# retab-dev/k-LLMs

Hardware: AMD Instinct MI355X
Metric: end_to_end_consensus_requests_per_s (higher is better)
Workload: dtype bf16; 1 GPU; model=llama-3-8b, n=5, mode=create, global_batch=24, seq_len=512, parallelism=dp1 tp1

## Files before the change

### kllms_amd/ops/hip/attn_decode.hip

```cpp

#include "common.h"

#define TKV ATTN_DECODE_TKV
#define NTHREADS 256
#define KLANES 4

#define PART_STRIDE 130

template <int GQA, bool FP8>
__global__ __launch_bounds__(NTHREADS) void attn_decode_partial_t(
    float* __restrict__ partials,
    const bf16_t* __restrict__ q,
    const char* __restrict__ k_cache,
    const char* __restrict__ v_cache,
    const float* __restrict__ k_scale,
    const float* __restrict__ v_scale,
    const int* __restrict__ block_tables,
    const int* __restrict__ context_lens,
    const int* __restrict__ skip_chunks,
    float scale, int num_kv_heads,
    int block_size, int max_blocks, int max_chunks, int q_tstride, int chunk_keys) {
  const int b = blockIdx.x;
  const int g_kv = blockIdx.y;
  const int chunk = blockIdx.z;
  if (skip_chunks != nullptr && chunk < skip_chunks[b]) return;
  const int L = context_lens[b];
  const int c0 = chunk * chunk_keys;
  if (c0 >= L && chunk > 0) return;
  const int c1 = min(L, c0 + chunk_keys);
  const int tid = threadIdx.x;

  extern __shared__ __attribute__((aligned(16))) char smem[];
  float* q_lds = reinterpret_cast<float*>(smem);
  float* s_lds = q_lds + GQA * 128;
  float* mstate = s_lds + GQA * TKV;
  float* lstate = mstate + 8;
  float* alpha_lds = lstate + 8;
  float* o_scratch = alpha_lds + 8;
  int64_t* rowoff = reinterpret_cast<int64_t*>(o_scratch + 4 * GQA * 128);
  float* ks_lds = reinterpret_cast<float*>(rowoff + TKV);
  float* vs_lds = ks_lds + TKV;

  for (int i = tid; i < GQA * 128; i += NTHREADS) {
    const int g = i >> 7, d = i & 127;
    const bf16_t* qp = q + (int64_t)b * q_tstride + (g_kv * GQA + g) * 128;
    q_lds[i] = bf16_to_f32(((const short*)qp)[d]) * scale;
  }
  if (tid < 8) { mstate[tid] = -INFINITY; lstate[tid] = 0.0f; }
  __syncthreads();

  float o_part[GQA][2];
#pragma unroll
  for (int g = 0; g < GQA; ++g) { o_part[g][0] = 0.f; o_part[g][1] = 0.f; }

  const int* bt = block_tables + (int64_t)b * max_blocks;

  for (int tile = c0; tile < c1; tile += TKV) {
    const int nkeys = min(TKV, c1 - tile);
    for (int i = tid; i < nkeys; i += NTHREADS) {
      const int gk = tile + i;
      const int64_t off = (((int64_t)bt[gk / block_size] * num_kv_heads + g_kv) * block_size +
                           (gk % block_size)) * 128;
      rowoff[i] = off;
      if constexpr (FP8) {
        ks_lds[i] = k_scale[off >> 7];
        vs_lds[i] = v_scale[off >> 7];
      }
    }
    __syncthreads();

    {
      constexpr int ELEMS = 128 / KLANES;
      constexpr int VECS = ELEMS / 8;
      const int kg = tid / KLANES;
      const int kl = tid % KLANES;
      for (int key0 = 0; key0 < nkeys; key0 += NTHREADS / KLANES) {
        const int key = key0 + kg;
        if (key < nkeys) {
          float af[ELEMS];
          if constexpr (FP8) {
            const u8x8_vec* kv8 = reinterpret_cast<const u8x8_vec*>(k_cache + rowoff[key]) + kl * VECS;
#pragma unroll
            for (int c = 0; c < VECS; ++c) {
              u8x8_vec kv = kv8[c];
#pragma unroll
              for (int j = 0; j < 8; ++j) af[c * 8 + j] = fp8_to_f32(kv[j]);
            }
          } else {
            const bf16x8_vec* kv8 =
                reinterpret_cast<const bf16x8_vec*>(k_cache + 2 * rowoff[key]) + kl * VECS;
#pragma unroll
            for (int c = 0; c < VECS; ++c) {
              bf16x8_vec kv = kv8[c];
#pragma unroll
              for (int j = 0; j < 8; ++j) af[c * 8 + j] = bf16_to_f32(kv[j]);
            }
          }
#pragma unroll
          for (int g = 0; g < GQA; ++g) {
            const float* qg = q_lds + g * 128 + kl * ELEMS;
            float acc = 0.f;
#pragma unroll
            for (int j = 0; j < ELEMS; ++j) acc += af[j] * qg[j];
#pragma unroll
            for (int off = KLANES / 2; off > 0; off >>= 1) acc += __shfl_xor(acc, off);
            if (kl == 0) s_lds[g * TKV + key] = FP8 ? acc * ks_lds[key] : acc;
          }
        }
      }
    }
    __syncthreads();

    {
      const int wave = tid >> 6;
      const int wlane = tid & 63;
      for (int g = wave; g < GQA; g += NTHREADS / 64) {
        float lm = -INFINITY;
        for (int i = wlane; i < nkeys; i += 64) lm = fmaxf(lm, s_lds[g * TKV + i]);
        const float tile_max = wave_reduce_max(lm);
        const float m_old = mstate[g];
        const float m_new = fmaxf(m_old, tile_max);
        const float alpha = (m_old == -INFINITY) ? 0.0f : __expf(m_old - m_new);
        float ls = 0.f;
        for (int i = wlane; i < nkeys; i += 64) {
          const float p = __expf(s_lds[g * TKV + i] - m_new);
          s_lds[g * TKV + i] = p;
          ls += p;
        }
        const float tile_sum = wave_reduce_sum(ls);
        if (wlane == 0) {
          alpha_lds[g] = alpha;
          mstate[g] = m_new;
          lstate[g] = lstate[g] * alpha + tile_sum;
        }
      }
    }
    __syncthreads();

    {
      const int kpart = tid >> 6;
      const int d0 = (tid & 63) * 2;
#pragma unroll
      for (int g = 0; g < GQA; ++g) {
        const float alpha = alpha_lds[g];
        o_part[g][0] *= alpha;
        o_part[g][1] *= alpha;
      }
      const int nk4 = (nkeys + 3) >> 2;
      const int kbeg = kpart * nk4;
      const int kend = min(nkeys, kbeg + nk4);
      int key = kbeg;
      for (; key + 4 <= kend; key += 4) {
        uint32_t pairs[4];
#pragma unroll
        for (int u = 0; u < 4; ++u) {
          if constexpr (FP8)
            pairs[u] = *reinterpret_cast<const unsigned short*>(v_cache + rowoff[key + u] + d0);
          else
            pairs[u] = *reinterpret_cast<const uint32_t*>(v_cache + 2 * (rowoff[key + u] + d0));
        }
#pragma unroll
        for (int u = 0; u < 4; ++u) {
          const float vs = FP8 ? vs_lds[key + u] : 1.0f;
          const float v0 = vs * (FP8 ? fp8_to_f32((unsigned char)(pairs[u] & 0xff))
                                     : bf16_to_f32((short)(pairs[u] & 0xffff)));
          const float v1 = vs * (FP8 ? fp8_to_f32((unsigned char)((pairs[u] >> 8) & 0xff))
                                     : bf16_to_f32((short)(pairs[u] >> 16)));
#pragma unroll
          for (int g = 0; g < GQA; ++g) {
            const float p = s_lds[g * TKV + key + u];
            o_part[g][0] += p * v0;
            o_part[g][1] += p * v1;
          }
        }
      }
      for (; key < kend; ++key) {
        uint32_t pair;
        if constexpr (FP8)
          pair = *reinterpret_cast<const unsigned short*>(v_cache + rowoff[key] + d0);
        else
          pair = *reinterpret_cast<const uint32_t*>(v_cache + 2 * (rowoff[key] + d0));
        const float vs = FP8 ? vs_lds[key] : 1.0f;
        const float v0 = vs * (FP8 ? fp8_to_f32((unsigned char)(pair & 0xff))
                                   : bf16_to_f32((short)(pair & 0xffff)));
        const float v1 = vs * (FP8 ? fp8_to_f32((unsigned char)((pair >> 8) & 0xff))
                                   : bf16_to_f32((short)(pair >> 16)));
#pragma unroll
        for (int g = 0; g < GQA; ++g) {
          const float p = s_lds[g * TKV + key];
          o_part[g][0] += p * v0;
          o_part[g][1] += p * v1;
        }
      }
    }
    __syncthreads();
  }

  {
    const int kpart = tid >> 6;
    const int d0 = (tid & 63) * 2;
#pragma unroll
    for (int g = 0; g < GQA; ++g) {
      o_scratch[((kpart * GQA + g) * 128) + d0] = o_part[g][0];
      o_scratch[((kpart * GQA + g) * 128) + d0 + 1] = o_part[g][1];
    }
  }
  __syncthreads();
  float* base = partials +
      ((((int64_t)b * num_kv_heads + g_kv) * max_chunks + chunk) * GQA) * PART_STRIDE;
  for (int i = tid; i < GQA * 128; i += NTHREADS) {
    const int g = i >> 7, d = i & 127;
    float acc = 0.f;
#pragma unroll
    for (int kp = 0; kp < 4; ++kp) acc += o_scratch[((kp * GQA + g) * 128) + d];
    base[g * PART_STRIDE + d] = acc;
  }
  if (tid < 8 && tid < GQA) {
    float* pg = base + tid * PART_STRIDE;
    pg[128] = mstate[tid];
    pg[129] = lstate[tid];
  }
}

extern "C" void launch_attn_decode_partial(
    float* partials, const bf16_t* q, const void* k_cache, const void* v_cache,
    const float* k_scale, const float* v_scale,
    const int* block_tables, const int* context_lens, const int* skip_chunks, float scale,
    int num_q_heads, int num_kv_heads, int block_size, int max_blocks,
    int max_chunks, int q_tstride, int chunk_keys, int B, int cache_fp8,
    hipStream_t stream) {
  const int gqa = num_q_heads / num_kv_heads;
  const dim3 grid(B, num_kv_heads, max_chunks);
  const size_t lds = (gqa * 128 + gqa * TKV + 24 + 4 * gqa * 128) * sizeof(float) +
                     TKV * sizeof(int64_t) + 2 * TKV * sizeof(float);
#define LAUNCH(G, F)                                                                  \
  hipLaunchKernelGGL((attn_decode_partial_t<G, F>), grid, dim3(NTHREADS), lds, stream, \
                     partials, q, (const char*)k_cache, (const char*)v_cache,          \
                     k_scale, v_scale,                                                 \
                     block_tables, context_lens, skip_chunks, scale, num_kv_heads,     \
                     block_size,                                                       \
                     max_blocks, max_chunks, q_tstride, chunk_keys)
#define DISPATCH(G) do { if (cache_fp8) LAUNCH(G, true); else LAUNCH(G, false); } while (0)
  switch (gqa) {
    case 1: DISPATCH(1); break;
    case 2: DISPATCH(2); break;
    case 4: DISPATCH(4); break;
    case 8: DISPATCH(8); break;
    default: DISPATCH(8); break;
  }
#undef DISPATCH
#undef LAUNCH
}

extern "C" __global__ void __launch_bounds__(64) attn_decode_reduce_kernel(
    bf16_t* __restrict__ out,
    const float* __restrict__ partials,
    const int* __restrict__ context_lens,
    int num_q_heads, int num_kv_heads, int max_chunks, int chunk_keys) {
  const int b = blockIdx.x;
  const int h = blockIdx.y;
  const int gqa = num_q_heads / num_kv_heads;
  const int g_kv = h / gqa;
  const int g = h % gqa;
  const int lane = threadIdx.x;
  const int nchunks = min(max_chunks, (context_lens[b] + chunk_keys - 1) / chunk_keys);

  const float* base = partials +
      ((((int64_t)b * num_kv_heads + g_kv) * max_chunks) * gqa + g) * PART_STRIDE;

  float m = -INFINITY;
  for (int c = 0; c < nchunks; ++c) m = fmaxf(m, base[(int64_t)c * gqa * PART_STRIDE + 128]);
  float l_tot = 0.0f;
  float acc0 = 0.0f, acc1 = 0.0f;
  for (int c = 0; c < nchunks; ++c) {
    const float* pc = base + (int64_t)c * gqa * PART_STRIDE;
    const float w = __expf(pc[128] - m);
    l_tot += pc[129] * w;
    acc0 += pc[lane * 2] * w;
    acc1 += pc[lane * 2 + 1] * w;
  }
  const float inv_l = (l_tot > 0.f) ? 1.0f / l_tot : 0.0f;
  bf16_t* op = out + (((int64_t)b * num_q_heads) + h) * 128;
  const uint32_t pair = ((uint32_t)(uint16_t)f32_to_bf16(acc1 * inv_l) << 16) |
                        (uint16_t)f32_to_bf16(acc0 * inv_l);
  *reinterpret_cast<uint32_t*>((short*)op + lane * 2) = pair;
}
```

Baseline: 31.08 req/s.

## Prefetch V rows in groups, swizzle block order, and use DPP quad reductions in decode attention

The P·V loop now loads V in groups of 16 keys and double-buffers them, so the next group's global loads are in flight while the current group's FMAs run. The blocks are also changed: the launch grid is linearised and batches are swizzled across groups of 8, the q load is vectorised and overlapped with first-tile rowoff staging (dropping one barrier), the key-lane reduction uses DPP instead of shuffles, and launch bounds request 4 blocks per SM. The extra registers for two 16-entry buffers may hurt occupancy or spill. Selective non-contracted multiply-add keeps rounding behaviour matched for the last GQA group.

```diff
diff --git a/kllms_amd/ops/hip/attn_decode.hip b/kllms_amd/ops/hip/attn_decode.hip
--- a/kllms_amd/ops/hip/attn_decode.hip
+++ b/kllms_amd/ops/hip/attn_decode.hip
@@ -1,14 +1,33 @@
 
 #include "common.h"
+
+#include <type_traits>
 
 #define TKV ATTN_DECODE_TKV
 #define NTHREADS 256
 #define KLANES 4
 
 #define PART_STRIDE 130
+#define V_GROUP 16
+
+static_assert(TKV == NTHREADS, "one rowoff slot per thread");
+
+__device__ __forceinline__ float quad_sum(float acc) {
+  acc += __int_as_float(__builtin_amdgcn_update_dpp(
+      0, __float_as_int(acc), 0x4E , 0xF, 0xF, false));
+  acc += __int_as_float(__builtin_amdgcn_update_dpp(
+      0, __float_as_int(acc), 0xB1 , 0xF, 0xF, false));
+  return acc;
+}
+
+__device__ __forceinline__ float mul_then_add(float p, float v, float o) {
+#pragma clang fp contract(off)
+  const float pv = p * v;
+  return o + pv;
+}
 
 template <int GQA, bool FP8>
-__global__ __launch_bounds__(NTHREADS) void attn_decode_partial_t(
+__global__ __launch_bounds__(NTHREADS, 4) void attn_decode_partial_t(
     float* __restrict__ partials,
     const bf16_t* __restrict__ q,
     const char* __restrict__ k_cache,
@@ -20,9 +39,25 @@
     const int* __restrict__ skip_chunks,
     float scale, int num_kv_heads,
     int block_size, int max_blocks, int max_chunks, int q_tstride, int chunk_keys) {
-  const int b = blockIdx.x;
-  const int g_kv = blockIdx.y;
-  const int chunk = blockIdx.z;
+  int b, g_kv, chunk;
+  {
+    const int nb = gridDim.x, ny = gridDim.y;
+    const int nb8 = nb / 8;
+    const int swizzled = nb8 * 8 * ny * (int)gridDim.z;
+    const int lin = blockIdx.x + nb * (blockIdx.y + ny * blockIdx.z);
+    int rest;
+    if (lin < swizzled) {
+      const int idx = lin / 8;
+      b = (lin % 8) * nb8 + idx % nb8;
+      rest = idx / nb8;
+    } else {
+      const int r = lin - swizzled, tail = nb - 8 * nb8;
+      b = 8 * nb8 + r % tail;
+      rest = r / tail;
+    }
+    g_kv = rest % ny;
+    chunk = rest / ny;
+  }
   if (skip_chunks != nullptr && chunk < skip_chunks[b]) return;
   const int L = context_lens[b];
   const int c0 = chunk * chunk_keys;
@@ -41,32 +76,45 @@
   float* ks_lds = reinterpret_cast<float*>(rowoff + TKV);
   float* vs_lds = ks_lds + TKV;
 
-  for (int i = tid; i < GQA * 128; i += NTHREADS) {
-    const int g = i >> 7, d = i & 127;
-    const bf16_t* qp = q + (int64_t)b * q_tstride + (g_kv * GQA + g) * 128;
-    q_lds[i] = bf16_to_f32(((const short*)qp)[d]) * scale;
+  const int* bt = block_tables + (int64_t)b * max_blocks;
+  auto stage_rowoff = [&](int tile, int nkeys) {
+    if (tid < nkeys) {
+      const int gk = tile + tid;
+      const int64_t off = (((int64_t)bt[gk / block_size] * num_kv_heads + g_kv) * block_size +
+                           (gk % block_size)) * 128;
+      rowoff[tid] = off;
+      if constexpr (FP8) {
+        ks_lds[tid] = k_scale[off >> 7];
+        vs_lds[tid] = v_scale[off >> 7];
+      }
+    }
+  };
+
+  {
+    const short* qrow =
+        reinterpret_cast<const short*>(q) + (int64_t)b * q_tstride + g_kv * GQA * 128;
+    const bool q_vec = (reinterpret_cast<uintptr_t>(qrow) & 15) == 0;
+    bf16x8_vec qv = {};
+    if (q_vec && tid < GQA * 16) qv = reinterpret_cast<const bf16x8_vec*>(qrow)[tid];
+    stage_rowoff(c0, min(TKV, c1 - c0));
+    if (q_vec) {
+      if (tid < GQA * 16) {
+#pragma unroll
+        for (int j = 0; j < 8; ++j) q_lds[tid * 8 + j] = bf16_to_f32(qv[j]) * scale;
+      }
+    } else {
+      for (int i = tid; i < GQA * 128; i += NTHREADS) q_lds[i] = bf16_to_f32(qrow[i]) * scale;
+    }
   }
   if (tid < 8) { mstate[tid] = -INFINITY; lstate[tid] = 0.0f; }
-  __syncthreads();
 
   float o_part[GQA][2];
 #pragma unroll
   for (int g = 0; g < GQA; ++g) { o_part[g][0] = 0.f; o_part[g][1] = 0.f; }
-
-  const int* bt = block_tables + (int64_t)b * max_blocks;
 
   for (int tile = c0; tile < c1; tile += TKV) {
     const int nkeys = min(TKV, c1 - tile);
-    for (int i = tid; i < nkeys; i += NTHREADS) {
-      const int gk = tile + i;
-      const int64_t off = (((int64_t)bt[gk / block_size] * num_kv_heads + g_kv) * block_size +
-                           (gk % block_size)) * 128;
-      rowoff[i] = off;
-      if constexpr (FP8) {
-        ks_lds[i] = k_scale[off >> 7];
-        vs_lds[i] = v_scale[off >> 7];
-      }
-    }
+    if (tile != c0) stage_rowoff(tile, nkeys);
     __syncthreads();
 
     {
@@ -102,8 +150,7 @@
             float acc = 0.f;
 #pragma unroll
             for (int j = 0; j < ELEMS; ++j) acc += af[j] * qg[j];
-#pragma unroll
-            for (int off = KLANES / 2; off > 0; off >>= 1) acc += __shfl_xor(acc, off);
+            acc = quad_sum(acc);
             if (kl == 0) s_lds[g * TKV + key] = FP8 ? acc * ks_lds[key] : acc;
           }
         }
@@ -138,59 +185,62 @@
     __syncthreads();
 
     {
-      const int kpart = tid >> 6;
-      const int d0 = (tid & 63) * 2;
 #pragma unroll
       for (int g = 0; g < GQA; ++g) {
         const float alpha = alpha_lds[g];
         o_part[g][0] *= alpha;
         o_part[g][1] *= alpha;
       }
+      const int kpart = __builtin_amdgcn_readfirstlane(tid >> 6);
+      const int d0 = (tid & 63) * 2;
       const int nk4 = (nkeys + 3) >> 2;
       const int kbeg = kpart * nk4;
       const int kend = min(nkeys, kbeg + nk4);
-      int key = kbeg;
-      for (; key + 4 <= kend; key += 4) {
-        uint32_t pairs[4];
-#pragma unroll
-        for (int u = 0; u < 4; ++u) {
+      auto load_v = [&](uint32_t (&dst)[V_GROUP], int key) {
+#pragma unroll
+        for (int u = 0; u < V_GROUP; ++u) {
+          const int64_t off = rowoff[min(key + u, kend - 1)];
           if constexpr (FP8)
-            pairs[u] = *reinterpret_cast<const unsigned short*>(v_cache + rowoff[key + u] + d0);
+            dst[u] = *reinterpret_cast<const unsigned short*>(v_cache + off + d0);
           else
-            pairs[u] = *reinterpret_cast<const uint32_t*>(v_cache + 2 * (rowoff[key + u] + d0));
-        }
-#pragma unroll
-        for (int u = 0; u < 4; ++u) {
-          const float vs = FP8 ? vs_lds[key + u] : 1.0f;
-          const float v0 = vs * (FP8 ? fp8_to_f32((unsigned char)(pairs[u] & 0xff))
-                                     : bf16_to_f32((short)(pairs[u] & 0xffff)));
-          const float v1 = vs * (FP8 ? fp8_to_f32((unsigned char)((pairs[u] >> 8) & 0xff))
-                                     : bf16_to_f32((short)(pairs[u] >> 16)));
-#pragma unroll
-          for (int g = 0; g < GQA; ++g) {
-            const float p = s_lds[g * TKV + key + u];
-            o_part[g][0] += p * v0;
-            o_part[g][1] += p * v1;
+            dst[u] = *reinterpret_cast<const uint32_t*>(v_cache + 2 * (off + d0));
+        }
+      };
+      auto fma_v = [&](auto full, const uint32_t (&pairs)[V_GROUP], int key) {
+#pragma unroll
+        for (int u = 0; u < V_GROUP; ++u) {
+          if (decltype(full)::value || key + u < kend) {
+            const bool blk4 = decltype(full)::value || key + (u | 3) < kend;
+            const float vs = FP8 ? vs_lds[key + u] : 1.0f;
+            const float v0 = vs * (FP8 ? fp8_to_f32((unsigned char)(pairs[u] & 0xff))
+                                       : bf16_to_f32((short)(pairs[u] & 0xffff)));
+            const float v1 = vs * (FP8 ? fp8_to_f32((unsigned char)((pairs[u] >> 8) & 0xff))
+                                       : bf16_to_f32((short)(pairs[u] >> 16)));
+#pragma unroll
+            for (int g = 0; g < GQA; ++g) {
+              const float p = s_lds[g * TKV + key + u];
+              if (g == GQA - 1 && blk4) {
+                o_part[g][0] = mul_then_add(p, v0, o_part[g][0]);
+                o_part[g][1] = mul_then_add(p, v1, o_part[g][1]);
+              } else {
+                o_part[g][0] = __builtin_fmaf(p, v0, o_part[g][0]);
+                o_part[g][1] = __builtin_fmaf(p, v1, o_part[g][1]);
+              }
+            }
           }
         }
-      }
-      for (; key < kend; ++key) {
-        uint32_t pair;
-        if constexpr (FP8)
-          pair = *reinterpret_cast<const unsigned short*>(v_cache + rowoff[key] + d0);
-        else
-          pair = *reinterpret_cast<const uint32_t*>(v_cache + 2 * (rowoff[key] + d0));
-        const float vs = FP8 ? vs_lds[key] : 1.0f;
-        const float v0 = vs * (FP8 ? fp8_to_f32((unsigned char)(pair & 0xff))
-                                   : bf16_to_f32((short)(pair & 0xffff)));
-        const float v1 = vs * (FP8 ? fp8_to_f32((unsigned char)((pair >> 8) & 0xff))
-                                   : bf16_to_f32((short)(pair >> 16)));
-#pragma unroll
-        for (int g = 0; g < GQA; ++g) {
-          const float p = s_lds[g * TKV + key];
-          o_part[g][0] += p * v0;
-          o_part[g][1] += p * v1;
-        }
+      };
+      if (kbeg < kend) {
+        uint32_t vcur[V_GROUP], vnxt[V_GROUP];
+        load_v(vcur, kbeg);
+        int key = kbeg;
+        for (; key + V_GROUP < kend; key += V_GROUP) {
+          load_v(vnxt, key + V_GROUP);
+          fma_v(std::true_type{}, vcur, key);
+#pragma unroll
+          for (int u = 0; u < V_GROUP; ++u) vcur[u] = vnxt[u];
+        }
+        fma_v(std::false_type{}, vcur, key);
       }
     }
     __syncthreads();
```

Result: faster. 32.20 req/s (median of 6 runs) (+3.6%).
